# e4s2022/e4s

Hardware: AMD Instinct MI355X
Metric: 1024^2 face-swap images/sec (higher is better)
Workload: dtype f32 operands as hi+lo bf16, 3 bf16 MFMAs per product, f32 accumulate (bf16x3) on the 3x3 convs whose launch fills the chip; exact f32 elsewhere; 1 GPU; E4S-core face swap at 1024^2 (2x Net3 encoder @256^2, style swap, 12 LocalMLPs, mask-guided StyleGAN2 generator K=13), BASELINE.json configs[3] shard: 8 swaps per GPU per step; per_gpu_batch=8, global_batch=8, out_size=1024, hip_graph=True, precision=as bf16x3 where the launch fills the chip (this batch), else exact fp32, parallelism=image-parallel x1

## Files before the change

e4s_amd/csrc/conv_bf16x3.hip:

```cpp
#include "common.h"
#include "few_tile_geom.h"
#include <stdlib.h>

namespace {

typedef __bf16 bf16x8 __attribute__((ext_vector_type(8)));
typedef float f32x8 __attribute__((ext_vector_type(8)));

constexpr int KC = 32;
constexpr int ROWB = 144;
constexpr int LO = 64;
constexpr int TW = 16, HALO_W = TW + 2;
constexpr int PBM = 256, PTH = 16, PHALO = (PTH + 2) * HALO_W;
constexpr int PNTHR = 512;

template <int BN_, int WM_, int WN_, int TPS_, int KCH_ = 32>
struct PCfg {
    static constexpr int BN = BN_, WM = WM_, WN = WN_, TPS = TPS_, KCH = KCH_;
    static constexpr int TM = PBM / (WM * 32), TN = BN / (WN * 32);
    static constexpr int ROWB = KCH == 32 ? 144 : 80;
    static constexpr int LO = KCH * 2;
    static constexpr int QG = KCH / 8;
    static constexpr int KSTEPS = KCH / 16;
    static constexpr int ITEMS = PHALO * QG;
    static constexpr int A_BYTES = PHALO * ROWB;
    static constexpr int NSTG = 9 / TPS;
    static constexpr int PIECE = ITEMS / NSTG;
    static constexpr int BPC = KCH / 4;
    static constexpr int BITEMS = TPS * BN * BPC;
    static constexpr int BJ = (BITEMS + PNTHR - 1) / PNTHR;
    static constexpr int B_BYTES = TPS * BN * ROWB;
    static_assert(KCH == 32 || KCH == 16, "chunk");
    static_assert(WM * WN * 64 == PNTHR && TM >= 1 && TN >= 1 && NSTG * TPS == 9, "wave layout");
    static_assert(PIECE * NSTG == ITEMS && PIECE <= PNTHR, "halo split");
};
using CfgL = PCfg<128, 4, 2, 1>;
using CfgL16 = PCfg<128, 4, 2, 3, 16>;
using CfgM = PCfg<64, 4, 2, 3>;
using CfgS = PCfg<32, 8, 1, 3>;

template <typename C, bool SHUF>
constexpr int plain_smem() {
    return 2 * C::A_BYTES + 2 * C::B_BYTES + 3 * PBM * 4 * (1 + (SHUF ? 4 : 1))
           + (SHUF ? 0 : C::WM * C::BN * 2 * 8);
}

__device__ __forceinline__ void split_store(unsigned char* dst, const f32x8 v, const int lo = LO) {
    const bf16x8 h = __builtin_convertvector(v, bf16x8);
    const f32x8 r = v - __builtin_convertvector(h, f32x8);
    const bf16x8 l = __builtin_convertvector(r, bf16x8);
    *reinterpret_cast<bf16x8*>(dst) = h;
    *reinterpret_cast<bf16x8*>(dst + lo) = l;
}

__device__ __forceinline__ f32x8 load8(const float* src) {
    const f32x4 lo4 = *reinterpret_cast<const f32x4*>(src);
    const f32x4 hi4 = *reinterpret_cast<const f32x4*>(src + 4);
    return f32x8{lo4[0], lo4[1], lo4[2], lo4[3], hi4[0], hi4[1], hi4[2], hi4[3]};
}

__global__ void splitk_epilogue_kernel(const e4s_conv_params p, const int ksplit, const int ycs, const int64_t hw,
                                       const int64_t n4);

inline void few_tiles_split(int64_t tiles, int nchunk, int& ksplit, int& cper) {
    ksplit = 1;
    cper = nchunk;
    if (tiles > 128 || nchunk < 4) return;
    int want = (int)((256 + tiles - 1) / tiles);
    if (want > nchunk / 2) want = nchunk / 2;
    if (want < 2) return;
    cper = (nchunk + want - 1) / want;
    ksplit = (nchunk + cper - 1) / cper;
}

inline bool region_pack_mode() {
    static const bool m = [] { const char* e = getenv("E4S_REGION_PACK"); return e ? atoi(e) != 0 : true; }();
    return m;
}

inline bool region_packed(const e4s_conv_params& p) {
    return region_pack_mode() && p.labels && (p.ncls == 1 || p.ncls == 4) && e4s_few_tile::pack_geom(p.Ha, p.Wa).n_img >= 2;
}

inline void region_split(const e4s_conv_params& p, int& ksplit, int& cper) {
    if (region_packed(p)) {
        const e4s_few_tile::PackGeom g = e4s_few_tile::pack_geom(p.Ha, p.Wa);
        e4s_few_tile::pack_split((int64_t)e4s_few_tile::pack_tiles(g, p.B) * p.ncls * (p.Cout / 128), p.Cin / 32, ksplit, cper);
        return;
    }
    const int64_t tiles = (int64_t)p.B * ((p.Ha + 15) / 16) * ((p.Wa + 15) / 16) * p.ncls * (p.Cout / 128);
    few_tiles_split(tiles, p.Cin / 32, ksplit, cper);
}

struct TileId {
    int tb, tyb, txb, n0, ks, c_lo, c_hi;
};

template <typename C, int XF, bool SHUF, int VAR = 0>
__global__ __launch_bounds__(PNTHR) void conv_bf16x3_kernel(const e4s_conv_params p, const int ntn, const int tx_n,
                                                            const int per_img, const int ntiles, const int ksplit,
                                                            const int cper) {
    constexpr int BM = PBM, BN = C::BN, NTHR = PNTHR, WN = C::WN, TM = C::TM, TN = C::TN, TH = PTH, TPS = C::TPS;
    constexpr int NSTG = C::NSTG, PIECE = C::PIECE, BITEMS = C::BITEMS, BJ = C::BJ;
    constexpr int A_BYTES = C::A_BYTES, B_BYTES = C::B_BYTES, NZ = SHUF ? 4 : 1;
    constexpr int KC = C::KCH, ROWB = C::ROWB, LO = C::LO, QG = C::QG, KSTEPS = C::KSTEPS, BPC = C::BPC, PITEMS = C::ITEMS;
    extern __shared__ __attribute__((aligned(16))) unsigned char smem[];
    unsigned char* sA = smem;
    unsigned char* sB = smem + 2 * A_BYTES;
    int* s_out = reinterpret_cast<int*>(sB + 2 * B_BYTES);
    float* s_nz = reinterpret_cast<float*>(s_out + 3 * BM);
    double* s_st = reinterpret_cast<double*>(s_nz + 3 * BM * NZ);

    const int tid = threadIdx.x;
    const int lane = tid & 63, wave = tid >> 6;
    const int li = lane & 31, kh = lane >> 5;
    const int wm = wave / WN, wn = wave % WN;
    const int G = gridDim.x;
    const int first = xcd_remap(blockIdx.x, G);

    const int nchunk = p.Cin / KC;
    auto decode = [&](int t0) -> TileId {
        TileId id;
        const int t = t0 / ksplit;
        id.ks = t0 - t * ksplit;
        id.c_lo = id.ks * cper;
        id.c_hi = min(id.c_lo + cper, nchunk);
        const int mt = t / ntn, nt = t - mt * ntn;
        id.n0 = nt * BN;
        id.tb = mt / per_img;
        const int rem = mt - id.tb * per_img;
        id.tyb = rem / tx_n;
        id.txb = rem - id.tyb * tx_n;
        return id;
    };
    auto fill_meta = [&](int buf, const TileId& id) {
        if (tid < BM) {
            const int ay = id.tyb * TH + tid / TW, ax = id.txb * TW + tid % TW;
            const bool valid = ay < p.Ha && ax < p.Wa;
            const int oy = ay * p.ostride, ox = ax * p.ostride;
            s_out[buf * BM + tid] = valid ? (id.tb * p.Ho + oy) * p.Wo + ox : -1;
#pragma unroll
            for (int ph = 0; ph < NZ; ++ph) {
                float nz = 0.f;
                if (valid && p.noise)
                    nz = p.noise_w[0] * p.noise[(int64_t)id.tb * p.noise_bstride + (int64_t)(oy + (ph >> 1)) * p.Wo + ox + (ph & 1)];
                s_nz[(buf * BM + tid) * NZ + ph] = nz;
            }
        }
    };

    const int ngemm = SHUF ? 4 * p.Cout : p.Cout;
    const unsigned char* wbytes = reinterpret_cast<const unsigned char*>(p.w);
    const size_t wrow = (size_t)p.Cin * 4;
    const size_t img_stride = (size_t)p.Hi * p.Wi * p.Cin;

    auto item_src = [&](const TileId& id, int item, bool& ok) -> size_t {
        const int h = item / QG, q = item % QG;
        const int hy = h / HALO_W, hx = h - hy * HALO_W;
        const int iy = id.tyb * TH + hy - 1, ix = id.txb * TW + hx - 1;
        ok = (unsigned)iy < (unsigned)p.Hi && (unsigned)ix < (unsigned)p.Wi;
// ... 569 lines not shown
                scale_split(raw, sv[tm][kk], ah, al);
                if (g + 1 < NG) raw = ldraw(g + 1);
            } else {
                const f32x8 v = raw * sv[tm][kk];
                if (g + 1 < NG) raw = ldraw(g + 1);
                ah = __builtin_convertvector(v, bf16x8);
                const f32x8 res = v - __builtin_convertvector(ah, f32x8);
                al = __builtin_convertvector(res, bf16x8);
            }
#pragma unroll
            for (int tn = 0; tn < TN; ++tn)
                acc[tm][tn] = __builtin_amdgcn_mfma_f32_32x32x16_bf16(al, bh[kk][tn], acc[tm][tn], 0, 0, 0);
#pragma unroll
            for (int tn = 0; tn < TN; ++tn)
                acc[tm][tn] = __builtin_amdgcn_mfma_f32_32x32x16_bf16(ah, bl[kk][tn], acc[tm][tn], 0, 0, 0);
#pragma unroll
            for (int tn = 0; tn < TN; ++tn)
                acc[tm][tn] = __builtin_amdgcn_mfma_f32_32x32x16_bf16(ah, bh[kk][tn], acc[tm][tn], 0, 0, 0);
        };
        mfma_group(0);
        issue_loads();
        if (NG == 4) mfma_group(1);
#pragma unroll
        for (int i = 0; i < 12; ++i) {
            __builtin_amdgcn_sched_group_barrier(0x008, 1, 0);
            __builtin_amdgcn_sched_group_barrier(0x126, 8, 0);
        }
        __builtin_amdgcn_sched_barrier(0);
        mfma_group(NG / 2);
        if (NG == 4) mfma_group(3);
#pragma unroll
        for (int i = 0; i < 12; ++i) {
            __builtin_amdgcn_sched_group_barrier(0x008, 1, 1);
            __builtin_amdgcn_sched_group_barrier(0x126, 6, 1);
        }
        __builtin_amdgcn_sched_barrier(0);

        if (more) {
            unsigned char* db = sB + ((s + 1) & 1) * B_BYTES + br0 * ROWB + bq;
#pragma unroll
            for (int j = 0; j < BJ; ++j) *reinterpret_cast<f32x4*>(db + BSTEP * j * ROWB) = pb[j];
        }
        if (have_next && piece_thr && item < XITEMS) {
            if (!it.ok) pa = f32x8{0.f, 0.f, 0.f, 0.f, 0.f, 0.f, 0.f, 0.f};
            store8(smem + ((chunk + 1) & 1) * it.bufstride + it.dst, pa);
        }
        __syncthreads();
        if (++tap == 9) { tap = 0; ++chunk; }
        if (++t1 == 9) { t1 = 0; ++c1; }
    }

    float* sD = reinterpret_cast<float*>(sA);
    if (p.out_scale && !PACK) {
        for (int t = tid; t < R * BN; t += NTHR) {
            const int r = t / BN, n = t - r * BN;
            sD[t] = p.out_scale[((size_t)tb * R + r) * p.Cout + n0 + n];
        }
        __syncthreads();
    }
    float bsv[TN];
#pragma unroll
    for (int tn = 0; tn < TN; ++tn) bsv[tn] = p.bias ? p.bias[n0 + (wn * TN + tn) * 32 + li] : 0.f;
    const float gain = (p.act == 1) ? p.gain : 1.f;
    const bool do_act = p.act != 0, scaled = p.out_scale != nullptr, raw = ksplit > 1;
    float* yo = raw ? p.splitk_ws + (size_t)ks * ((size_t)p.B * p.Ho * p.Wo * p.Cout) : p.y;
#pragma unroll
    for (int tm = 0; tm < TM; ++tm) {
#pragma unroll
        for (int g = 0; g < 4; ++g) {
            float v[TN][4];
#pragma unroll
            for (int i = 0; i < 4; ++i) {
                const int r = 4 * g + i;
                const int row = (wm * TM + tm) * 32 + i + 8 * g + 4 * kh;
                const float nz = s_nz[row];
                const float* drow = PACK ? p.out_scale + (size_t)s_grp[row] * p.Cout + n0 : sD + s_grp[row] * BN;
#pragma unroll
                for (int tn = 0; tn < TN; ++tn) {
                    const int ncol = (wn * TN + tn) * 32 + li;
                    float t = acc[tm][tn][r] * (scaled ? drow[ncol] : 1.f);
                    if (!raw) {
                        t += nz + bsv[tn];
                        if (do_act) t = (t > 0.f ? t : t * p.alpha) * gain;
                    }
                    v[tn][i] = t;
                }
            }
#pragma unroll
            for (int tn = 0; tn < TN; ++tn) quad_transpose4(v[tn][0], v[tn][1], v[tn][2], v[tn][3], li);
            const int off = s_out[(wm * TM + tm) * 32 + (li & 3) + 8 * g + 4 * kh];
            if (off >= 0) {
#pragma unroll
                for (int tn = 0; tn < TN; ++tn)
                    *reinterpret_cast<f32x4*>(yo + (size_t)off * p.Cout + n0 + (wn * TN + tn) * 32 + (li & ~3)) =
                        f32x4{v[tn][0], v[tn][1], v[tn][2], v[tn][3]};
            }
        }
    }
    if (!SCAN) return;
    scan_b += gridDim.x;
    __syncthreads();
  }
}

template <int WN_, int SPL>
int launch_region_v(const e4s_conv_params& p, const int* only_flagged, hipStream_t st) {
    const bool pack = region_packed(p);
    if (pack && only_flagged) return (int)hipErrorInvalidValue;
    auto kern = pack ? conv_bf16x3_region_kernel<WN_, SPL, false, true>
                     : only_flagged ? conv_bf16x3_region_kernel<WN_, SPL, true> : conv_bf16x3_region_kernel<WN_, SPL, false>;
    static std::atomic<uint64_t> smem_set[3] = {{0}, {0}, {0}};
    if (int e = e4s_ensure_dyn_smem(reinterpret_cast<const void*>(kern), SMEM_REGION, smem_set[pack ? 2 : only_flagged ? 1 : 0])) return e;
    const int ntn = p.Cout / BN;
    const e4s_few_tile::PackGeom geo = e4s_few_tile::pack_geom(p.Ha, p.Wa);
    const int tx_n = pack ? geo.n_img : (p.Wa + TW - 1) / TW, per_img = pack ? 1 : ((p.Ha + TH - 1) / TH) * tx_n;
    const int tiles_per_cls = pack ? e4s_few_tile::pack_tiles(geo, p.B) : p.B * per_img;
    int ksplit, cper;
    region_split(p, ksplit, cper);
    if (ksplit > 1 && !p.splitk_ws) return (int)hipErrorInvalidValue;
    const int64_t blocks = (int64_t)tiles_per_cls * p.ncls * ntn * ksplit;
    if (blocks <= 0) return 0;
    if (blocks >= (1ll << 31)) return (int)hipErrorInvalidValue;
    const unsigned grid = only_flagged ? (unsigned)(blocks < 256 ? blocks : 256) : (unsigned)blocks;
    hipLaunchKernelGGL(kern, dim3(grid), dim3(NTHR), SMEM_REGION, st, p, ntn, tx_n, per_img, tiles_per_cls,
                       ksplit, cper, only_flagged, (int)blocks);
    E4S_CHECK_LAUNCH();
    if (ksplit > 1) {
        e4s_conv_params q = p;
        q.out_scale = nullptr;
        const int64_t n4 = (int64_t)p.B * p.Ho * p.Wo * (p.Cout / 4);
        hipLaunchKernelGGL(splitk_epilogue_kernel, dim3((unsigned)((n4 + 255) / 256)), dim3(256), 0, st, q, ksplit, p.Cout,
                           (int64_t)p.Ho * p.Wo, n4);
        E4S_CHECK_LAUNCH();
    }
    return 0;
}

int launch_region(const e4s_conv_params& p, const int* only_flagged, hipStream_t st) {
#ifdef E4S_ABLATIONS
    static const int v = [] { const char* e = getenv("E4S_REGION_VAR"); return e ? atoi(e) : -1; }();
    switch (v) {
        case 0: return launch_region_v<2, 0>(p, only_flagged, st);
        case 1: return launch_region_v<2, 1>(p, only_flagged, st);
        case 2: return launch_region_v<1, 0>(p, only_flagged, st);
        default: break;
    }
#endif
    return launch_region_v<1, 1>(p, only_flagged, st);
}

constexpr int GA_BYTES = BM * ROWB;
constexpr int SMEM_GATHER = 2 * GA_BYTES + 2 * B_BYTES + BM * 4;

__global__ __launch_bounds__(NTHR) void conv_bf16x3_gather_kernel(const e4s_conv_params p, const int ntn,
                                                                  const int npix, const int ntile, const int ksplit,
                                                                  const int cper) {
    extern __shared__ __attribute__((aligned(16))) unsigned char smem[];
    unsigned char* sA = smem;
    unsigned char* sB = smem + 2 * GA_BYTES;
    int* s_out = reinterpret_cast<int*>(sB + 2 * B_BYTES);

    const int tid = threadIdx.x;
    const int lane = tid & 63, wave = tid >> 6;
    const int li = lane & 31, kh = lane >> 5;
    const int wm = wave / WN, wn = wave % WN;
    const int logical = xcd_remap(blockIdx.x, gridDim.x);
    const int ks = logical / ntile, tile = logical - ks * ntile;
    const int mt = tile / ntn, nt = tile - mt * ntn;
    const int n0 = nt * BN;
    const int hw = p.Ha * p.Wa;
    const int c_lo = ks * cper, c_hi = min(p.Cin / KC, c_lo + cper);

    if (tid < BM) {
        const int a = mt * BM + tid;
        s_out[tid] = a < npix ? a : -1;
    }
    const int aq = tid & 3, ar0 = tid >> 2;
    int a_base[2], a_yx[2];
#pragma unroll
    for (int j = 0; j < 2; ++j) {
        const int a = mt * BM + ar0 + 128 * j;
        const bool valid = a < npix;
        const int aa = valid ? a : 0;
        const int b = aa / hw, rem = aa - b * hw;
        const int ay = rem / p.Wa, ax = rem - ay * p.Wa;
        const int by = ay * p.istride, bx = ax * p.istride;
        a_base[j] = (b * p.Hi + by) * p.Wi + bx;
        a_yx[j] = valid ? ((by << 16) | bx) : 0x7fff7fff;
    }
    const int ntaps = p.ntaps, nstage = ntaps * (c_hi - c_lo);
    const unsigned char* wbytes = reinterpret_cast<const unsigned char*>(p.w);
    const size_t wrow = (size_t)p.Cin * 4;
    const int bq = (tid & 7) * 16, br0 = tid >> 3;
    const int ncols = min(BN, p.Cout - n0);
    const bool cols_live = wn * TN * 32 < ncols;
    const f32x8 zero8 = {0.f, 0.f, 0.f, 0.f, 0.f, 0.f, 0.f, 0.f};

    struct Pref {
        f32x4 b[BJ];
        f32x8 a[2];
        unsigned ok;
    };
    auto fetch = [&](Pref& P, int tap, int chunk) {
        const unsigned char* wp = wbytes + ((size_t)tap * p.Cout + n0) * wrow + (size_t)chunk * 128 + bq;
#pragma unroll
        for (int j = 0; j < BJ; ++j) P.b[j] = *reinterpret_cast<const f32x4*>(wp + (size_t)min(br0 + BSTEP * j, ncols - 1) * wrow);
        const int oy = ((ntaps == 9) ? tap / 3 - 1 : 0) + p.tap_shift, ox = ((ntaps == 9) ? tap % 3 - 1 : 0) + p.tap_shift;
        unsigned okm = 0;
#pragma unroll
        for (int j = 0; j < 2; ++j) {
            const int iy = (a_yx[j] >> 16) + oy, ix = (a_yx[j] & 0xffff) + ox;
            const bool ok = (unsigned)iy < (unsigned)p.Hi && (unsigned)ix < (unsigned)p.Wi;
            const size_t off = ok ? (size_t)(a_base[j] + oy * p.Wi + ox) * p.Cin : 0;
            P.a[j] = load8(p.x + off + chunk * KC + aq * 8);
            okm |= (ok ? 1u : 0u) << j;
        }
        P.ok = okm;
    };
    auto store = [&](const Pref& P, int buf) {
        unsigned char* db = sB + buf * B_BYTES + br0 * ROWB + bq;
#pragma unroll
        for (int j = 0; j < BJ; ++j) *reinterpret_cast<f32x4*>(db + BSTEP * j * ROWB) = P.b[j];
#pragma unroll
        for (int j = 0; j < 2; ++j)
            split_store(sA + buf * GA_BYTES + (ar0 + 128 * j) * ROWB + aq * 16, ((P.ok >> j) & 1u) ? P.a[j] : zero8);
    };

    int arow[TM], brow[TN];
#pragma unroll
    for (int tm = 0; tm < TM; ++tm) arow[tm] = ((wm * TM + tm) * 32 + li) * ROWB + kh * 16;
#pragma unroll
    for (int tn = 0; tn < TN; ++tn) brow[tn] = ((wn * TN + tn) * 32 + li) * ROWB + kh * 16;
    f32x16 acc[TM][TN];
#pragma unroll
    for (int tm = 0; tm < TM; ++tm)
#pragma unroll
        for (int tn = 0; tn < TN; ++tn)
#pragma unroll
            for (int r = 0; r < 16; ++r) acc[tm][tn][r] = 0.f;

    Pref P;
    fetch(P, 0, c_lo);
    store(P, 0);
    __syncthreads();
    int t1 = 0, c1 = c_lo;
    if (++t1 == ntaps) { t1 = 0; ++c1; }
    for (int s = 0; s < nstage; ++s) {
        const unsigned char* Ab = sA + (s & 1) * GA_BYTES;
        const unsigned char* Bb = sB + (s & 1) * B_BYTES;
        const bool more = s + 1 < nstage;
        bf16x8 bh[2][TN], bl[2][TN], ah[2], al[2];
        auto ldB = [&](int kk) {
#pragma unroll
            for (int tn = 0; tn < TN; ++tn) {
                bh[kk][tn] = *reinterpret_cast<const bf16x8*>(Bb + brow[tn] + kk * 32);
                bl[kk][tn] = *reinterpret_cast<const bf16x8*>(Bb + brow[tn] + kk * 32 + LO);
            }
        };
        auto ldA = [&](int g, int slot) {
            const int kk = g / TM, tm = g % TM;
            ah[slot] = *reinterpret_cast<const bf16x8*>(Ab + arow[tm] + kk * 32);
            al[slot] = *reinterpret_cast<const bf16x8*>(Ab + arow[tm] + kk * 32 + LO);
        };
        auto mfma_group = [&](int g) {
            const int kk = g / TM, tm = g % TM, cur = g & 1;
            if (g + 1 < 2 * TM) ldA(g + 1, cur ^ 1);
#pragma unroll
            for (int tn = 0; tn < TN; ++tn)
                acc[tm][tn] = __builtin_amdgcn_mfma_f32_32x32x16_bf16(al[cur], bh[kk][tn], acc[tm][tn], 0, 0, 0);
#pragma unroll
            for (int tn = 0; tn < TN; ++tn)
                acc[tm][tn] = __builtin_amdgcn_mfma_f32_32x32x16_bf16(ah[cur], bl[kk][tn], acc[tm][tn], 0, 0, 0);
#pragma unroll
            for (int tn = 0; tn < TN; ++tn)
                acc[tm][tn] = __builtin_amdgcn_mfma_f32_32x32x16_bf16(ah[cur], bh[kk][tn], acc[tm][tn], 0, 0, 0);
        };
        if (!cols_live) {
            fetch(P, more ? t1 : 0, more ? c1 : c_lo);
            if (more) store(P, (s + 1) & 1);
            __syncthreads();
            if (++t1 == ntaps) { t1 = 0; ++c1; }
            continue;
        }
        ldB(0);
        ldA(0, 0);
        __builtin_amdgcn_sched_barrier(0);
        mfma_group(0);
        fetch(P, more ? t1 : 0, more ? c1 : c_lo);
        ldB(1);
        mfma_group(1);
#pragma unroll
        for (int i = 0; i < 12; ++i) {
            __builtin_amdgcn_sched_group_barrier(0x008, 1, 0);
            __builtin_amdgcn_sched_group_barrier(0x126, 10, 0);
        }
        __builtin_amdgcn_sched_barrier(0);
        mfma_group(2);
        __builtin_amdgcn_sched_barrier(0);
        mfma_group(3);
        __builtin_amdgcn_sched_barrier(0);
        if (more) store(P, (s + 1) & 1);
        __syncthreads();
        if (++t1 == ntaps) { t1 = 0; ++c1; }
    }

    const bool raw = ksplit > 1;
    float bsv[TN], slp[TN];
#pragma unroll
    for (int tn = 0; tn < TN; ++tn) {
        const int col = n0 + min((wn * TN + tn) * 32 + li, ncols - 1);
        bsv[tn] = (p.bias && !raw) ? p.bias[col] : 0.f;
        slp[tn] = (p.act == 2 && !raw) ? p.slope[col] : p.alpha;
    }
    const float gain = (p.act == 1) ? p.gain : 1.f;
    const bool do_act = p.act != 0 && !raw;
    const bool stats = p.stats_ws != nullptr;
    double st_s[TN], st_q[TN];
#pragma unroll
    for (int tn = 0; tn < TN; ++tn) st_s[tn] = st_q[tn] = 0.0;
    const int gycs = p.y_cstride ? p.y_cstride : p.Cout;
    const bool wide = (gycs & 3) == 0;
    float* const yout = raw ? p.splitk_ws + (size_t)ks * ((size_t)npix * gycs) : p.y;
#pragma unroll
    for (int tm = 0; tm < TM; ++tm) {
#pragma unroll
        for (int g = 0; g < 4; ++g) {
            float v[TN][4];
#pragma unroll
            for (int i = 0; i < 4; ++i) {
                const int r = 4 * g + i;
                const bool live = s_out[(wm * TM + tm) * 32 + i + 8 * g + 4 * kh] >= 0;
#pragma unroll
                for (int tn = 0; tn < TN; ++tn) {
                    float t = acc[tm][tn][r] + bsv[tn];
                    if (do_act) t = (t > 0.f ? t : t * slp[tn]) * gain;
                    v[tn][i] = t;
                    if (stats && live) { st_s[tn] += (double)t; st_q[tn] += (double)t * (double)t; }
                }
            }
            if (wide) {
#pragma unroll
                for (int tn = 0; tn < TN; ++tn) quad_transpose4(v[tn][0], v[tn][1], v[tn][2], v[tn][3], li);
                const int off = s_out[(wm * TM + tm) * 32 + (li & 3) + 8 * g + 4 * kh];
                if (off >= 0 && cols_live) {
#pragma unroll
                    for (int tn = 0; tn < TN; ++tn)
                        *reinterpret_cast<f32x4*>(yout + (size_t)off * gycs + n0 + (wn * TN + tn) * 32 + (li & ~3)) =
                            f32x4{v[tn][0], v[tn][1], v[tn][2], v[tn][3]};
                }
            } else {
#pragma unroll
                for (int i = 0; i < 4; ++i) {
                    const int off = s_out[(wm * TM + tm) * 32 + i + 8 * g + 4 * kh];
                    if (off < 0 || !cols_live) continue;
#pragma unroll
                    for (int tn = 0; tn < TN; ++tn) yout[(size_t)off * gycs + n0 + (wn * TN + tn) * 32 + li] = v[tn][i];
                }
            }
        }
    }
    if (stats) {
        double* s_st = reinterpret_cast<double*>(sA);
#pragma unroll
        for (int tn = 0; tn < TN; ++tn) {
            st_s[tn] += __shfl_xor(st_s[tn], 32, 64);
            st_q[tn] += __shfl_xor(st_q[tn], 32, 64);
            if (kh == 0) {
                const int col = (wn * TN + tn) * 32 + li;
                s_st[(wm * BN + col) * 2] = st_s[tn];
                s_st[(wm * BN + col) * 2 + 1] = st_q[tn];
            }
        }
        __syncthreads();
        if (tid < ncols) {
            double a = 0.0, q = 0.0;
#pragma unroll
            for (int j = 0; j < NTHR / 64 / WN; ++j) { a += s_st[(j * BN + tid) * 2]; q += s_st[(j * BN + tid) * 2 + 1]; }
            const int tiles_per_img = hw / BM;
            const int b = mt / tiles_per_img, tile_in_img = mt - b * tiles_per_img;
            double* slot = p.stats_ws + (((size_t)b * p.Cout + n0 + tid) * p.stats_slots + tile_in_img) * 2;
            slot[0] = a;
            slot[1] = q;
        }
    }
}

void gather_split(const e4s_conv_params& p, int& ksplit, int& cper) {
    ksplit = 1;
    cper = p.Cin / KC;
    const int ycs = p.y_cstride ? p.y_cstride : p.Cout;
    if (p.ntaps != 9 || p.Cin < 256 || p.Cin % KC || (ycs & 3)) return;
    const int64_t tiles = (((int64_t)p.B * p.Ha * p.Wa + BM - 1) / BM) * ((p.Cout + BN - 1) / BN);
    if (tiles <= 0 || tiles > 64) return;
    few_tiles_split(tiles, p.Cin / KC, ksplit, cper);
}

int launch_gather(const e4s_conv_params& p, hipStream_t st) {
    auto kern = conv_bf16x3_gather_kernel;
    static std::atomic<uint64_t> smem_set{0};
    if (int e = e4s_ensure_dyn_smem(reinterpret_cast<const void*>(kern), SMEM_GATHER, smem_set)) return e;
    const int ntn = (p.Cout + BN - 1) / BN;
    const int64_t npix = (int64_t)p.B * p.Ha * p.Wa;
    if (npix <= 0) return 0;
    if (npix * ntn >= (1ll << 31)) return (int)hipErrorInvalidValue;
    const int64_t ntile = ((npix + BM - 1) / BM) * ntn;
    int ksplit, cper;
    gather_split(p, ksplit, cper);
    if (ksplit > 1 && (!p.splitk_ws || p.stats_ws)) return (int)hipErrorInvalidValue;
    hipLaunchKernelGGL(kern, dim3((unsigned)(ntile * ksplit)), dim3(NTHR), SMEM_GATHER, st, p, ntn, (int)npix, (int)ntile, ksplit, cper);
    E4S_CHECK_LAUNCH();
    return ksplit > 1 ? e4s_splitk_epilogue(p, ksplit, st) : 0;
}

__global__ void split_bf16x2_kernel(const float* __restrict__ w, unsigned short* __restrict__ out, int64_t n8,
                                    int cin) {
    const int64_t i = (int64_t)blockIdx.x * blockDim.x + threadIdx.x;
    if (i >= n8) return;
    const int g8 = cin / 8;
    const int64_t row = i / g8;
    const int c = (int)(i - row * g8) * 8;
    const f32x4 a = *reinterpret_cast<const f32x4*>(w + row * cin + c);
    const f32x4 b = *reinterpret_cast<const f32x4*>(w + row * cin + c + 4);
    const f32x8 v = {a[0], a[1], a[2], a[3], b[0], b[1], b[2], b[3]};
    const bf16x8 h = __builtin_convertvector(v, bf16x8);
    const f32x8 r = v - __builtin_convertvector(h, f32x8);
    const bf16x8 l = __builtin_convertvector(r, bf16x8);
    unsigned short* d = out + row * (int64_t)cin * 2 + (c / 32) * 64 + (c % 32);
    *reinterpret_cast<bf16x8*>(d) = h;
    *reinterpret_cast<bf16x8*>(d + 32) = l;
}

__global__ void splitk_epilogue_kernel(const e4s_conv_params p, const int ksplit, const int ycs, const int64_t hw,
                                       const int64_t n4) {
    const int C4 = p.Cout / 4;
    const int64_t i = (int64_t)blockIdx.x * blockDim.x + threadIdx.x;
    if (i >= n4) return;
    const int c = (int)(i % C4) * 4;
    const int64_t pix = i / C4;
    const int64_t b = pix / hw;
    const size_t slab = (size_t)p.B * hw * ycs;
    const float* src = p.splitk_ws + (size_t)pix * ycs + c;
    f32x4 v = *reinterpret_cast<const f32x4*>(src);
    for (int k = 1; k < ksplit; ++k) v += *reinterpret_cast<const f32x4*>(src + (size_t)k * slab);
    float nz = 0.f;
    if (p.noise) nz = p.noise_w[0] * p.noise[b * p.noise_bstride + (pix - b * hw)];
    const float gain = (p.act == 1) ? p.gain : 1.f;
#pragma unroll
    for (int e = 0; e < 4; ++e) {
        float t = v[e] * (p.out_scale ? p.out_scale[b * p.Cout + c + e] : 1.f) + nz + (p.bias ? p.bias[c + e] : 0.f);
        if (p.act) t = (t > 0.f ? t : t * (p.act == 2 ? p.slope[c + e] : p.alpha)) * gain;
        v[e] = t;
    }
    *reinterpret_cast<f32x4*>(p.y + (size_t)pix * ycs + c) = v;
}

void plain_split(const e4s_conv_params& p, int ntn, int& ksplit, int& cper) {
    const int64_t tiles = (int64_t)p.B * ((p.Ha + PTH - 1) / PTH) * ((p.Wa + TW - 1) / TW) * ntn;
    few_tiles_split(tiles, p.Cin / KC, ksplit, cper);
}

int num_cus() {
    static int cus[64] = {0};
    int dev = 0;
    if (hipGetDevice(&dev) != hipSuccess) return 256;
    if (!cus[dev & 63]) {
        hipDeviceProp_t prop;
        cus[dev & 63] = (hipGetDeviceProperties(&prop, dev) == hipSuccess && prop.multiProcessorCount > 0)
                            ? prop.multiProcessorCount : 256;
    }
    return cus[dev & 63];
}

template <typename C, int XF, bool SHUF, int VAR = 0>
int launch(const e4s_conv_params& p, hipStream_t st) {
    auto kern = conv_bf16x3_kernel<C, XF, SHUF, VAR>;
    constexpr int SMEM = plain_smem<C, SHUF>();
    static_assert(SMEM <= 160 * 1024, "LDS budget");
    static std::atomic<uint64_t> smem_set{0};
    if (int e = e4s_ensure_dyn_smem(reinterpret_cast<const void*>(kern), SMEM, smem_set)) return e;
    const int ngemm = SHUF ? 4 * p.Cout : p.Cout;
    const int ntn = ngemm / C::BN;
    const int tx_n = (p.Wa + TW - 1) / TW, per_img = ((p.Ha + PTH - 1) / PTH) * tx_n;
    int ksplit, cper;
    plain_split(p, ngemm / C::BN, ksplit, cper);
    cper *= 32 / C::KCH;
    if (ksplit > 1 && !p.splitk_ws) return (int)hipErrorInvalidValue;
    const int64_t ntiles = (int64_t)p.B * per_img * ntn * ksplit;
    if (ntiles <= 0) return 0;
    if (ntiles >= (1ll << 31)) return (int)hipErrorInvalidValue;
    const int grid = (int)(ntiles < num_cus() ? ntiles : num_cus());
    hipLaunchKernelGGL(kern, dim3((unsigned)grid), dim3(PNTHR), SMEM, st, p, ntn, tx_n, per_img, (int)ntiles, ksplit, cper);
    E4S_CHECK_LAUNCH();
    if (ksplit > 1) {
        const int ycs = p.y_cstride ? p.y_cstride : p.Cout;
        const int64_t npix = (int64_t)p.B * p.Ho * p.Wo;
        const int64_t n4 = npix * (p.Cout / 4);
        hipLaunchKernelGGL(splitk_epilogue_kernel, dim3((unsigned)((n4 + 255) / 256)), dim3(256), 0, st, p, ksplit, ycs,
                           (int64_t)p.Ho * p.Wo, n4);
        E4S_CHECK_LAUNCH();
    }
    return 0;
}

template <typename C, bool SHUF>
int launch_xf(const e4s_conv_params& p, hipStream_t st) {
    if (p.in_stats) return SHUF ? (int)hipErrorInvalidValue : launch<C, 2, false>(p, st);
    return p.in_scale ? launch<C, 1, SHUF>(p, st) : launch<C, 0, SHUF>(p, st);
}

}

int e4s_launch_region_select(const e4s_conv_params& p, const int* only_flagged, hipStream_t st) {
    return launch_region(p, only_flagged, st);
}
void e4s_region_split_policy(const e4s_conv_params& p, int& ksplit, int& cper) { region_split(p, ksplit, cper); }
bool e4s_region_packed(const e4s_conv_params& p) { return region_packed(p); }

extern "C" int e4s_conv_bf16x3_f32(const e4s_conv_params* pp, void* stream) {
    const e4s_conv_params& p = *pp;
    const bool up = (p.ncls == 4);
    if (p.istride == 2 || p.ntaps == 1) {
        if (p.Cin % KC || (p.Cout % BN && p.Cout != 64) || (p.ntaps != 9 && p.ntaps != 1) || p.ncls != 1 || p.ostride != 1 || p.tiles ||
            p.labels || p.in_scale || p.out_scale || p.in_stats || p.noise || p.Ho != p.Ha || p.Wo != p.Wa ||
            p.Hi >= 32767 || p.Wi >= 32767 || (p.Ha - 1) * p.istride >= p.Hi || (p.Wa - 1) * p.istride >= p.Wi ||
            p.tap_shift < 0 || p.tap_shift > 1 ||
            (p.stats_ws && (p.act != 0 || (p.Ha * p.Wa) % BM || p.stats_slots != (p.Ha * p.Wa) / BM)))
            return (int)hipErrorInvalidValue;
        return launch_gather(p, as_stream(stream));
    }
    if (p.Cin % KC || p.Cout % 32 || p.ntaps != 9 || (p.ncls != 1 && !up) || p.istride != 1 ||
        p.ostride != (up ? 2 : 1) || p.tiles || p.noise_per_channel || p.Ha != p.Hi || p.Wa != p.Wi ||
        p.Ho != p.Hi * p.ostride || p.Wo != p.Wi * p.ostride || (p.in_stats && p.in_scale))
        return (int)hipErrorInvalidValue;
    if (p.stats_ws && (p.labels || up || p.act != 0 || p.noise || p.out_scale ||
                       p.stats_slots != ((p.Ha + PTH - 1) / PTH) * ((p.Wa + TW - 1) / TW)))
        return (int)hipErrorInvalidValue;
    hipStream_t st = as_stream(stream);
    if (p.labels) {
        if (p.y_cstride || !p.in_scale || p.in_stats || p.act == 2 || p.Cout % BN || p.groups_per_batch < 1 || p.groups_per_batch > MAXR)
            return (int)hipErrorInvalidValue;
        return launch_region(p, nullptr, st);
    }
#ifdef E4S_ABLATIONS
    static const int abl = [] { const char* e = getenv("E4S_BF16X3_ABL"); return e ? atoi(e) : 0; }();
    if (abl && !up && p.Cout % 128 == 0 && !p.in_stats && !p.in_scale) {
        switch (abl) {
            case 1: return launch<CfgL, 0, false, 1>(p, st);
            case 2: return launch<CfgL, 0, false, 2>(p, st);
            case 3: return launch<CfgL, 0, false, 3>(p, st);
            case 4: return launch<CfgL, 0, false, 4>(p, st);
            case 5: return launch<CfgL, 0, false, 5>(p, st);
// ... 61 lines not shown
```

Baseline: 484.0 images/s.

## Deepen gather conv pipeline to two register stages with interleaved split-store

Restructures the bf16x3 gather conv main loop to prefetch two stages ahead into alternating register sets. It interleaves the global fetch, the hi/lo bf16 split and the LDS stores one by one between individual MFMAs, using fine-grained sched_group_barriers. It also swaps __syncthreads for an LDS-only fence barrier and precomputes weight row offsets with an incrementally advanced weight pointer. The goal is to hide global load latency and the split arithmetic behind MFMA work, at the cost of more registers (a second prefetch set) and possible occupancy or spill risk.

```diff
diff --git a/e4s_amd/csrc/conv_bf16x3.hip b/e4s_amd/csrc/conv_bf16x3.hip
--- a/e4s_amd/csrc/conv_bf16x3.hip
+++ b/e4s_amd/csrc/conv_bf16x3.hip
@@ -1,11 +1,15 @@
 #include "common.h"
 #include "few_tile_geom.h"
 #include <stdlib.h>
+#include <type_traits>
 
 namespace {
 
 typedef __bf16 bf16x8 __attribute__((ext_vector_type(8)));
 typedef float f32x8 __attribute__((ext_vector_type(8)));
+typedef float f32x2 __attribute__((ext_vector_type(2)));
+typedef __bf16 bf16x2 __attribute__((ext_vector_type(2)));
+typedef unsigned u32x4 __attribute__((ext_vector_type(4)));
 
 constexpr int KC = 32;
 constexpr int ROWB = 144;
@@ -881,6 +885,13 @@
 constexpr int GA_BYTES = BM * ROWB;
 constexpr int SMEM_GATHER = 2 * GA_BYTES + 2 * B_BYTES + BM * 4;
 
+__device__ __forceinline__ void lds_barrier() {
+    __builtin_amdgcn_fence(__ATOMIC_RELEASE, "workgroup", "local");
+    __builtin_amdgcn_s_barrier();
+    __builtin_amdgcn_fence(__ATOMIC_ACQUIRE, "workgroup", "local");
+}
+
+template <int VAR = 0>
 __global__ __launch_bounds__(NTHR) void conv_bf16x3_gather_kernel(const e4s_conv_params p, const int ntn,
                                                                   const int npix, const int ntile, const int ksplit,
                                                                   const int cper) {
@@ -905,7 +916,7 @@
         s_out[tid] = a < npix ? a : -1;
     }
     const int aq = tid & 3, ar0 = tid >> 2;
-    int a_base[2], a_yx[2];
+    int a_base[2], a_y[2], a_x[2];
 #pragma unroll
     for (int j = 0; j < 2; ++j) {
         const int a = mt * BM + ar0 + 128 * j;
@@ -915,7 +926,8 @@
         const int ay = rem / p.Wa, ax = rem - ay * p.Wa;
         const int by = ay * p.istride, bx = ax * p.istride;
         a_base[j] = (b * p.Hi + by) * p.Wi + bx;
-        a_yx[j] = valid ? ((by << 16) | bx) : 0x7fff7fff;
+        a_y[j] = valid ? by : 0x7fff;
+        a_x[j] = valid ? bx : 0x7fff;
     }
     const int ntaps = p.ntaps, nstage = ntaps * (c_hi - c_lo);
     const unsigned char* wbytes = reinterpret_cast<const unsigned char*>(p.w);
@@ -923,36 +935,55 @@
     const int bq = (tid & 7) * 16, br0 = tid >> 3;
     const int ncols = min(BN, p.Cout - n0);
     const bool cols_live = wn * TN * 32 < ncols;
-    const f32x8 zero8 = {0.f, 0.f, 0.f, 0.f, 0.f, 0.f, 0.f, 0.f};
+    size_t b_off[BJ];
+#pragma unroll
+    for (int j = 0; j < BJ; ++j) b_off[j] = (size_t)min(br0 + BSTEP * j, ncols - 1) * wrow + bq;
 
     struct Pref {
         f32x4 b[BJ];
         f32x8 a[2];
-        unsigned ok;
-    };
-    auto fetch = [&](Pref& P, int tap, int chunk) {
-        const unsigned char* wp = wbytes + ((size_t)tap * p.Cout + n0) * wrow + (size_t)chunk * 128 + bq;
-#pragma unroll
-        for (int j = 0; j < BJ; ++j) P.b[j] = *reinterpret_cast<const f32x4*>(wp + (size_t)min(br0 + BSTEP * j, ncols - 1) * wrow);
+        unsigned ok[2];
+    };
+    auto fetch_b = [&](Pref& P, const unsigned char* wp) {
+#pragma unroll
+        for (int j = 0; j < BJ; ++j) P.b[j] = *reinterpret_cast<const f32x4*>(wp + b_off[j]);
+    };
+    auto fetch_a0 = [&](Pref& P, int j, int tap, int& idx) {
         const int oy = ((ntaps == 9) ? tap / 3 - 1 : 0) + p.tap_shift, ox = ((ntaps == 9) ? tap % 3 - 1 : 0) + p.tap_shift;
-        unsigned okm = 0;
+        const int iy = a_y[j] + oy, ix = a_x[j] + ox;
+        const unsigned ok = (unsigned)((unsigned)iy < (unsigned)p.Hi) & (unsigned)((unsigned)ix < (unsigned)p.Wi);
+        idx = (a_base[j] + oy * p.Wi + ox) & (0 - (int)ok);
+        P.ok[j] = ok;
+        asm volatile("" : "+v"(idx));
+    };
+    auto fetch_a1 = [&](Pref& P, int j, int chunk, int idx) {
+        P.a[j] = load8(p.x + (size_t)idx * p.Cin + chunk * KC + aq * 8);
+    };
+    auto split_hi = [&](const Pref& P, int j, int q, float& v0, float& v1, unsigned& hi) {
+        v0 = P.ok[j] ? P.a[j][2 * q] : 0.f;
+        v1 = P.ok[j] ? P.a[j][2 * q + 1] : 0.f;
+        hi = __builtin_bit_cast(unsigned, __builtin_convertvector(f32x2{v0, v1}, bf16x2));
+        asm volatile("" : "+v"(hi));
+    };
+    auto split_lo = [&](float v0, float v1, unsigned hi, unsigned& lo) {
+        const float h0 = __builtin_bit_cast(float, hi << 16), h1 = __builtin_bit_cast(float, hi & 0xffff0000u);
+        lo = __builtin_bit_cast(unsigned, __builtin_convertvector(f32x2{v0 - h0, v1 - h1}, bf16x2));
+        asm volatile("" : "+v"(lo));
+    };
+    auto store_b = [&](const Pref& P, int buf, int j) {
+        *reinterpret_cast<f32x4*>(sB + buf * B_BYTES + (br0 + BSTEP * j) * ROWB + bq) = P.b[j];
+    };
+    auto store_a = [&](int buf, int j, int half, const unsigned (&w)[4]) {
+        *reinterpret_cast<u32x4*>(sA + buf * GA_BYTES + (ar0 + 128 * j) * ROWB + aq * 16 + half * LO) = u32x4{w[0], w[1], w[2], w[3]};
+    };
+    auto fetch = [&](Pref& P, const unsigned char* wp, int tap, int chunk) {
+        fetch_b(P, wp);
 #pragma unroll
         for (int j = 0; j < 2; ++j) {
-            const int iy = (a_yx[j] >> 16) + oy, ix = (a_yx[j] & 0xffff) + ox;
-            const bool ok = (unsigned)iy < (unsigned)p.Hi && (unsigned)ix < (unsigned)p.Wi;
-            const size_t off = ok ? (size_t)(a_base[j] + oy * p.Wi + ox) * p.Cin : 0;
-            P.a[j] = load8(p.x + off + chunk * KC + aq * 8);
-            okm |= (ok ? 1u : 0u) << j;
-        }
-        P.ok = okm;
-    };
-    auto store = [&](const Pref& P, int buf) {
-        unsigned char* db = sB + buf * B_BYTES + br0 * ROWB + bq;
-#pragma unroll
-        for (int j = 0; j < BJ; ++j) *reinterpret_cast<f32x4*>(db + BSTEP * j * ROWB) = P.b[j];
-#pragma unroll
-        for (int j = 0; j < 2; ++j)
-            split_store(sA + buf * GA_BYTES + (ar0 + 128 * j) * ROWB + aq * 16, ((P.ok >> j) & 1u) ? P.a[j] : zero8);
+            int idx;
+            fetch_a0(P, j, tap, idx);
+            fetch_a1(P, j, chunk, idx);
+        }
     };
 
     int arow[TM], brow[TN];
@@ -968,70 +999,111 @@
 #pragma unroll
             for (int r = 0; r < 16; ++r) acc[tm][tn][r] = 0.f;
 
-    Pref P;
-    fetch(P, 0, c_lo);
-    store(P, 0);
-    __syncthreads();
-    int t1 = 0, c1 = c_lo;
-    if (++t1 == ntaps) { t1 = 0; ++c1; }
-    for (int s = 0; s < nstage; ++s) {
-        const unsigned char* Ab = sA + (s & 1) * GA_BYTES;
-        const unsigned char* Bb = sB + (s & 1) * B_BYTES;
-        const bool more = s + 1 < nstage;
+    Pref R0, R1;
+    int t2 = 0, c2 = c_lo;
+    const size_t wtap = (size_t)p.Cout * wrow;
+    const unsigned char* const w0 = wbytes + (size_t)n0 * wrow + (size_t)c_lo * 128;
+    const unsigned char* w2 = w0;
+    auto advance = [&]() {
+        ++t2;
+        const bool wrap = t2 == ntaps;
+        t2 = wrap ? 0 : t2;
+        c2 += wrap ? 1 : 0;
+        w2 = wrap ? w2 - (size_t)(ntaps - 1) * wtap + 128 : w2 + wtap;
+    };
+    fetch(R0, w0, 0, c_lo);
+    advance();
+    fetch(R1, nstage > 1 ? w2 : w0, nstage > 1 ? t2 : 0, nstage > 1 ? c2 : c_lo);
+    advance();
+#pragma unroll
+    for (int j = 0; j < BJ; ++j) store_b(R0, 0, j);
+#pragma unroll
+    for (int j = 0; j < 2; ++j) {
+        unsigned hw[4], lw[4];
+#pragma unroll
+        for (int q = 0; q < 4; ++q) {
+            float v0, v1;
+            split_hi(R0, j, q, v0, v1, hw[q]);
+            split_lo(v0, v1, hw[q], lw[q]);
+        }
+        store_a(0, j, 0, hw);
+        store_a(0, j, 1, lw);
+    }
+    lds_barrier();
+
+    auto stage = [&](auto par_c, auto live_c, const int s) {
+        constexpr int PAR = decltype(par_c)::value;
+        constexpr bool LIVE = decltype(live_c)::value;
+        const unsigned char* Ab = sA + PAR * GA_BYTES;
+        const unsigned char* Bb = sB + PAR * B_BYTES;
+        Pref& Rf = PAR ? R1 : R0;
+        const Pref& Rs = PAR ? R0 : R1;
+        const bool more2 = s + 2 < nstage;
+        const int tap = more2 ? t2 : 0, chunk = more2 ? c2 : c_lo;
+        const unsigned char* const wp = more2 ? w2 : w0;
         bf16x8 bh[2][TN], bl[2][TN], ah[2], al[2];
-        auto ldB = [&](int kk) {
-#pragma unroll
-            for (int tn = 0; tn < TN; ++tn) {
-                bh[kk][tn] = *reinterpret_cast<const bf16x8*>(Bb + brow[tn] + kk * 32);
-                bl[kk][tn] = *reinterpret_cast<const bf16x8*>(Bb + brow[tn] + kk * 32 + LO);
-            }
+        auto ldB = [&](int kk, int tn) {
+            bh[kk][tn] = *reinterpret_cast<const bf16x8*>(Bb + brow[tn] + kk * 32);
+            bl[kk][tn] = *reinterpret_cast<const bf16x8*>(Bb + brow[tn] + kk * 32 + LO);
         };
         auto ldA = [&](int g, int slot) {
             const int kk = g / TM, tm = g % TM;
             ah[slot] = *reinterpret_cast<const bf16x8*>(Ab + arow[tm] + kk * 32);
             al[slot] = *reinterpret_cast<const bf16x8*>(Ab + arow[tm] + kk * 32 + LO);
         };
-        auto mfma_group = [&](int g) {
-            const int kk = g / TM, tm = g % TM, cur = g & 1;
-            if (g + 1 < 2 * TM) ldA(g + 1, cur ^ 1);
-#pragma unroll
-            for (int tn = 0; tn < TN; ++tn)
-                acc[tm][tn] = __builtin_amdgcn_mfma_f32_32x32x16_bf16(al[cur], bh[kk][tn], acc[tm][tn], 0, 0, 0);
-#pragma unroll
-            for (int tn = 0; tn < TN; ++tn)
-                acc[tm][tn] = __builtin_amdgcn_mfma_f32_32x32x16_bf16(ah[cur], bl[kk][tn], acc[tm][tn], 0, 0, 0);
-#pragma unroll
-            for (int tn = 0; tn < TN; ++tn)
-                acc[tm][tn] = __builtin_amdgcn_mfma_f32_32x32x16_bf16(ah[cur], bh[kk][tn], acc[tm][tn], 0, 0, 0);
-        };
-        if (!cols_live) {
-            fetch(P, more ? t1 : 0, more ? c1 : c_lo);
-            if (more) store(P, (s + 1) & 1);
-            __syncthreads();
-            if (++t1 == ntaps) { t1 = 0; ++c1; }
-            continue;
-        }
-        ldB(0);
-        ldA(0, 0);
+        if (LIVE) {
+#pragma unroll
+            for (int tn = 0; tn < TN; ++tn) ldB(0, tn);
+            ldA(0, 0);
+        }
         __builtin_amdgcn_sched_barrier(0);
-        mfma_group(0);
-        fetch(P, more ? t1 : 0, more ? c1 : c_lo);
-        ldB(1);
-        mfma_group(1);
-#pragma unroll
-        for (int i = 0; i < 12; ++i) {
-            __builtin_amdgcn_sched_group_barrier(0x008, 1, 0);
-            __builtin_amdgcn_sched_group_barrier(0x126, 10, 0);
-        }
-        __builtin_amdgcn_sched_barrier(0);
-        mfma_group(2);
-        __builtin_amdgcn_sched_barrier(0);
-        mfma_group(3);
-        __builtin_amdgcn_sched_barrier(0);
-        if (more) store(P, (s + 1) & 1);
-        __syncthreads();
-        if (++t1 == ntaps) { t1 = 0; ++c1; }
-    }
+        int idx = 0;
+        float v0 = 0.f, v1 = 0.f;
+        unsigned hw[2][4], lw[2][4];
+#pragma unroll
+        for (int k = 0; k < 6 * 2 * TM; ++k) {
+            const int g = k / 6, i = k % 6, kk = g / TM, tm = g % TM, cur = g & 1, prod = i >> 1, tn = i & 1;
+            if (LIVE) {
+                acc[tm][tn] = prod == 0 ? __builtin_amdgcn_mfma_f32_32x32x16_bf16(al[cur], bh[kk][tn], acc[tm][tn], 0, 0, 0)
+                            : prod == 1 ? __builtin_amdgcn_mfma_f32_32x32x16_bf16(ah[cur], bl[kk][tn], acc[tm][tn], 0, 0, 0)
+                                        : __builtin_amdgcn_mfma_f32_32x32x16_bf16(ah[cur], bh[kk][tn], acc[tm][tn], 0, 0, 0);
+                if (k > 0) {
+                    __builtin_amdgcn_sched_group_barrier(0x008, 1, 0);
+                    __builtin_amdgcn_sched_group_barrier(0x092, 16, 0);
+                }
+                if (i == 0 && g + 1 < 2 * TM) ldA(g + 1, cur ^ 1);
+                if (k == 1 || k == 2) ldB(1, k - 1);
+            }
+            if (VAR != 2) {
+                if (k == 7) fetch_b(Rf, wp);
+                if (k == 1 || k == 3) fetch_a0(Rf, k >> 1, tap, idx);
+                if (k == 2 || k == 4) fetch_a1(Rf, (k >> 1) - 1, chunk, idx);
+            }
+            if (VAR != 1) {
+                if (k == 5 || k == 6) store_b(Rs, PAR ^ 1, k - 5);
+                if (k >= 5 && k <= 20) {
+                    const int j = (k - 5) >> 3, q = ((k - 5) >> 1) & 3;
+                    if ((k - 5) & 1) split_lo(v0, v1, hw[j][q], lw[j][q]);
+                    else split_hi(Rs, j, q, v0, v1, hw[j][q]);
+                }
+                if (k == 13 || k == 21) store_a(PAR ^ 1, (k - 13) >> 3, 0, hw[(k - 13) >> 3]);
+                if (k == 14 || k == 22) store_a(PAR ^ 1, (k - 14) >> 3, 1, lw[(k - 14) >> 3]);
+            }
+            __builtin_amdgcn_sched_barrier(0);
+        }
+        lds_barrier();
+        advance();
+    };
+    auto stages = [&](auto live_c) {
+        int s = 0;
+        for (; s + 1 < nstage; s += 2) {
+            stage(std::integral_constant<int, 0>{}, live_c, s);
+            stage(std::integral_constant<int, 1>{}, live_c, s + 1);
+        }
+        if (s < nstage) stage(std::integral_constant<int, 0>{}, live_c, s);
+    };
+    if (cols_live) stages(std::true_type{});
+    else stages(std::false_type{});
 
     const bool raw = ksplit > 1;
     float bsv[TN], slp[TN];
@@ -1125,7 +1197,12 @@
 }
 
 int launch_gather(const e4s_conv_params& p, hipStream_t st) {
-    auto kern = conv_bf16x3_gather_kernel;
+    auto kern = conv_bf16x3_gather_kernel<0>;
+#ifdef E4S_ABLATIONS
+    static const int v = [] { const char* e = getenv("E4S_GATHER_VAR"); return e ? atoi(e) : 0; }();
+    if (v == 1) kern = conv_bf16x3_gather_kernel<1>;
+    if (v == 2) kern = conv_bf16x3_gather_kernel<2>;
+#endif
     static std::atomic<uint64_t> smem_set{0};
     if (int e = e4s_ensure_dyn_smem(reinterpret_cast<const void*>(kern), SMEM_GATHER, smem_set)) return e;
     const int ntn = (p.Cout + BN - 1) / BN;
```

Result: no change. 488.7 images/s, median of 6 (+1.0%).
